# DelphinusLab/halo2-gpu-specific

Hardware: AMD Instinct MI355X
Metric: NTT Fr-ops/s @ k=24 (forward+inverse 2^24 BN254 Fr NTT; MSM G1-adds/s under 'msm') (higher is better)
Workload: dtype u32x8 (254-bit Montgomery, integer)

## Files before the change

### halo2-gpu-specific_amd/csrc/field.hpp

```cpp
#pragma once
#ifdef __HIPCC_RTC__
typedef unsigned char uint8_t;
typedef unsigned short uint16_t;
typedef unsigned int uint32_t;
typedef unsigned long uint64_t;
typedef int int32_t;
typedef long int64_t;
#else
#include <hip/hip_runtime.h>
#include <stdint.h>
#endif

namespace h2 {

struct FrParams {
    static constexpr uint32_t MOD[8] = {0xf0000001u, 0x43e1f593u, 0x79b97091u, 0x2833e848u,
                                        0x8181585du, 0xb85045b6u, 0xe131a029u, 0x30644e72u};
    static constexpr uint32_t MOD2[8] = {0xe0000002u, 0x87c3eb27u, 0xf372e122u, 0x5067d090u,
                                         0x0302b0bau, 0x70a08b6du, 0xc2634053u, 0x60c89ce5u};
    static constexpr uint32_t NMOD[8] = {0x0fffffffu, 0xbc1e0a6cu, 0x86468f6eu, 0xd7cc17b7u,
                                         0x7e7ea7a2u, 0x47afba49u, 0x1ece5fd6u, 0xcf9bb18du};
    static constexpr uint32_t PINV256[8] = {0xefffffffu, 0xc2e1f593u, 0x4c6911b3u, 0x6586864bu,
                                         0x99062391u, 0xe39a9828u, 0x0d8341b2u, 0x73f82f1du};
    static constexpr uint32_t INV = 0xefffffffu;
// ... 280 lines not shown
    u.l[0] = add_co(d.l[0], P::MOD2[0], cb);
#pragma unroll
    for (int i = 2; i < 8; i++) {
        d.l[i] = subb_co(a.l[i], b.l[i], ca);
        u.l[i - 1] = addc_co(d.l[i - 1], P::MOD2[i - 1], cb);
    }
    u.l[7] = addc_co(d.l[7], P::MOD2[7], cb);
#else
    uint64_t borrow = 0, c = 0;
#pragma unroll
    for (int i = 0; i < 8; i++) {
        uint64_t t = (uint64_t)a.l[i] - b.l[i] - borrow;
        d.l[i] = (uint32_t)t;
        borrow = (t >> 32) & 1;
    }
#pragma unroll
    for (int i = 0; i < 8; i++) {
        c += (uint64_t)d.l[i] + P::MOD2[i];
        u.l[i] = (uint32_t)c;
        c >>= 32;
    }
#endif
    return u;
}
template <class P>
H2_DEV Fp<P> fp_lazy_add_red(const Fp<P>& a, const Fp<P>& b) {
#ifdef H2_ASM_CHAINS
    Fp<P> s, t, r;
    uint64_t ca, cb;
    s.l[0] = add_co(a.l[0], b.l[0], ca);
    s.l[1] = addc_co(a.l[1], b.l[1], ca);
    t.l[0] = sub_co(s.l[0], P::MOD2[0], cb);
#pragma unroll
    for (int i = 2; i < 8; i++) {
        s.l[i] = addc_co(a.l[i], b.l[i], ca);
        t.l[i - 1] = subb_co(s.l[i - 1], P::MOD2[i - 1], cb);
    }
    t.l[7] = subb_co(s.l[7], P::MOD2[7], cb);
#pragma unroll
    for (int i = 0; i < 8; i++) r.l[i] = sel_co(t.l[i], s.l[i], cb);
    return r;
#else
    return fp_lazy_red2p(fp_lazy_add(a, b));
#endif
}
template <class P>
H2_DEV Fp<P> fp_lazy_sub_red(const Fp<P>& a, const Fp<P>& b) {
#ifdef H2_ASM_CHAINS
    Fp<P> d, u, r;
    uint64_t ca, cb;
    d.l[0] = sub_co(a.l[0], b.l[0], ca);
    d.l[1] = subb_co(a.l[1], b.l[1], ca);
    u.l[0] = add_co(d.l[0], P::MOD2[0], cb);
#pragma unroll
    for (int i = 2; i < 8; i++) {
        d.l[i] = subb_co(a.l[i], b.l[i], ca);
        u.l[i - 1] = addc_co(d.l[i - 1], P::MOD2[i - 1], cb);
    }
    u.l[7] = addc_co(d.l[7], P::MOD2[7], cb);
#pragma unroll
    for (int i = 0; i < 8; i++) r.l[i] = sel_co(d.l[i], u.l[i], ca);
    return r;
#else
    return fp_lazy_red2p(fp_lazy_sub(a, b));
#endif
}
template <class P>
H2_DEV Fp<P> fp_lazy_canon(const Fp<P>& a) {
    return fp_reduce_once(fp_lazy_red2p(a));
}

template <int CL>
struct alignas(16) FpChunk {
    uint32_t w[64 / CL];
};

H2_DEV void mad_acc(uint64_t& lo, uint32_t& hi, uint32_t a, uint32_t b) {
#if defined(H2_PORTABLE_MUL) || !defined(__HIP_DEVICE_COMPILE__)
    uint64_t p = (uint64_t)a * b;
    uint64_t s = lo + p;
    hi += (s < p) ? 1u : 0u;
    lo = s;
#else
    uint64_t carry;
    asm("v_mad_u64_u32 %0, %1, %2, %3, %0" : "+v"(lo), "=s"(carry) : "v"(a), "v"(b));
    asm("v_addc_co_u32 %0, %1, %0, 0, %1" : "+v"(hi), "+s"(carry));
#endif
}

template <class P>
__device__ __forceinline__ Fp<P> fp_mul_dev(const Fp<P>& a, const Fp<P>& b);
template <class P>
__device__ __forceinline__ Fp<P> fp_sqr_dev(const Fp<P>& a);
template <class P>
__device__ __forceinline__ Fp<P> fp_mul2_dev(const Fp<P>& a, const Fp<P>& b, const Fp<P>& c, const Fp<P>& d);
template <class P>
__device__ __forceinline__ Fp<P> fp_mul_wide_dev(const Fp<P>& a, const Fp<P>& b);
template <class P>
__device__ __forceinline__ Fp<P> fp_mul_const_dev(const Fp<P>& a, const Fp<P>& w, const Fp<P>& wq);
template <class P, int CL>
__device__ __forceinline__ Fp<P> fp_mul_chunk_dev(const Fp<P>& a, const FpChunk<CL>& t);
#if defined(__HIP_DEVICE_COMPILE__) && !defined(H2_PORTABLE_MUL)
#include "fp_mul_gen.hpp"
#endif

template <class P>
H2_DEV Fp<P> fp_mul(const Fp<P>& a, const Fp<P>& b) {
#if !defined(__HIP_DEVICE_COMPILE__)
    {
        typedef unsigned __int128 u128;
        uint64_t x[4], y[4], p[4];
        for (int i = 0; i < 4; i++) {
            x[i] = (uint64_t)a.l[2 * i] | ((uint64_t)a.l[2 * i + 1] << 32);
            y[i] = (uint64_t)b.l[2 * i] | ((uint64_t)b.l[2 * i + 1] << 32);
            p[i] = (uint64_t)P::MOD[2 * i] | ((uint64_t)P::MOD[2 * i + 1] << 32);
        }
        uint64_t inv = p[0];
        for (int i = 0; i < 6; i++) inv *= 2 - p[0] * inv;
        inv = 0 - inv;
        uint64_t t[6] = {0, 0, 0, 0, 0, 0};
        for (int i = 0; i < 4; i++) {
            u128 c = 0;
            for (int j = 0; j < 4; j++) {
                c += (u128)t[j] + (u128)x[j] * y[i];
                t[j] = (uint64_t)c;
                c >>= 64;
            }
            c += t[4];
            t[4] = (uint64_t)c;
            t[5] = (uint64_t)(c >> 64);
            const uint64_t m = t[0] * inv;
            c = ((u128)t[0] + (u128)m * p[0]) >> 64;
            for (int j = 1; j < 4; j++) {
                c += (u128)t[j] + (u128)m * p[j];
                t[j - 1] = (uint64_t)c;
                c >>= 64;
            }
            c += t[4];
            t[3] = (uint64_t)c;
            t[4] = t[5] + (uint64_t)(c >> 64);
        }
        Fp<P> r;
        for (int i = 0; i < 4; i++) {
            r.l[2 * i] = (uint32_t)t[i];
            r.l[2 * i + 1] = (uint32_t)(t[i] >> 32);
        }
        return fp_reduce_once(r);
    }
#elif !defined(H2_PORTABLE_MUL)
    return fp_mul_dev(a, b);
#endif
    Fp<P> r;
    uint64_t lo = 0;
    uint32_t hi = 0;
    uint32_t m[8];
#pragma unroll
    for (int i = 0; i < 8; i++) {
#pragma unroll
        for (int j = 0; j <= i; j++) mad_acc(lo, hi, a.l[j], b.l[i - j]);
#pragma unroll
        for (int j = 0; j < i; j++) mad_acc(lo, hi, m[j], P::MOD[i - j]);
        m[i] = (uint32_t)lo * P::INV;
        mad_acc(lo, hi, m[i], P::MOD[0]);
        lo = (lo >> 32) | ((uint64_t)hi << 32);
        hi = 0;
    }
#pragma unroll
    for (int i = 8; i < 16; i++) {
#pragma unroll
        for (int j = i - 7; j < 8; j++) mad_acc(lo, hi, a.l[j], b.l[i - j]);
#pragma unroll
        for (int j = i - 7; j < 8; j++) mad_acc(lo, hi, m[j], P::MOD[i - j]);
        r.l[i - 8] = (uint32_t)lo;
        lo = (lo >> 32) | ((uint64_t)hi << 32);
        hi = 0;
    }
    return fp_reduce_once(r);
}

template <class P>
H2_DEV Fp<P> fp_sqr(const Fp<P>& a) {
#if defined(__HIP_DEVICE_COMPILE__) && !defined(H2_PORTABLE_MUL) && !defined(H2_NO_SQR)
    return fp_sqr_dev(a);
#else
    return fp_mul(a, a);
#endif
}

template <class P>
H2_DEV Fp<P> fp_mul2(const Fp<P>& a, const Fp<P>& b, const Fp<P>& c, const Fp<P>& d) {
#if defined(__HIP_DEVICE_COMPILE__) && !defined(H2_PORTABLE_MUL) && !defined(H2_NO_MUL2)
    return fp_mul2_dev(a, b, c, d);
#else
    return fp_add(fp_mul(a, b), fp_mul(c, d));
#endif
}

template <class P>
H2_DEV Fp<P> fp_mul_wide(const Fp<P>& a, const Fp<P>& b) {
#if defined(__HIP_DEVICE_COMPILE__) && !defined(H2_PORTABLE_MUL)
    return fp_mul_wide_dev(a, b);
#else
    Fp<P> r;
    uint64_t lo = 0;
    uint32_t hi = 0;
    uint32_t m[8];
    for (int i = 0; i < 8; i++) {
        for (int j = 0; j <= i; j++) mad_acc(lo, hi, a.l[j], b.l[i - j]);
        for (int j = 0; j < i; j++) mad_acc(lo, hi, m[j], P::MOD[i - j]);
        m[i] = (uint32_t)lo * P::INV;
        mad_acc(lo, hi, m[i], P::MOD[0]);
        lo = (lo >> 32) | ((uint64_t)hi << 32);
        hi = 0;
    }
    for (int i = 8; i < 16; i++) {
        for (int j = i - 7; j < 8; j++) mad_acc(lo, hi, a.l[j], b.l[i - j]);
        for (int j = i - 7; j < 8; j++) mad_acc(lo, hi, m[j], P::MOD[i - j]);
        r.l[i - 8] = (uint32_t)lo;
        lo = (lo >> 32) | ((uint64_t)hi << 32);
        hi = 0;
    }
    return r;
#endif
}

template <class P>
H2_DEV Fp<P> fp_mul_const(const Fp<P>& x, const Fp<P>& w, const Fp<P>& wq) {
#if defined(__HIP_DEVICE_COMPILE__) && !defined(H2_PORTABLE_MUL)
    Fp<P> r = fp_mul_const_dev(x, w, wq);
    if (__builtin_expect(r.l[7] >= P::MOD2[7], 0)) r = fp_lazy_red2p(r);
    return r;
#else
    uint32_t q[8];
    {
        uint64_t lo = 0;
        uint32_t hi = 0;
        for (int i = 0; i < 15; i++) {
            for (int j = (i > 7 ? i - 7 : 0); j <= (i < 7 ? i : 7); j++) mad_acc(lo, hi, x.l[j], wq.l[i - j]);
            if (i >= 8) q[i - 8] = (uint32_t)lo;
            lo = (lo >> 32) | ((uint64_t)hi << 32);
            hi = 0;
        }
        q[7] = (uint32_t)lo;
    }
    Fp<P> r;
    uint64_t lo = 0;
    uint32_t hi = 0;
    for (int i = 0; i < 8; i++) {
        for (int j = 0; j <= i; j++) {
            mad_acc(lo, hi, x.l[j], w.l[i - j]);
            mad_acc(lo, hi, q[j], P::NMOD[i - j]);
        }
        r.l[i] = (uint32_t)lo;
        lo = (lo >> 32) | ((uint64_t)hi << 32);
        hi = 0;
    }
    return r;
#endif
}
template <class P>
H2_DEV void fp_const_pair(const Fp<P>& w_mont, Fp<P>& w_plain, Fp<P>& wq) {
    w_plain = fp_from_mont(w_mont);
    uint64_t lo = 0;
    uint32_t hi = 0;
    for (int i = 0; i < 8; i++) {
        for (int j = 0; j <= i; j++) mad_acc(lo, hi, w_mont.l[j], P::PINV256[i - j]);
        wq.l[i] = (uint32_t)lo;
        lo = (lo >> 32) | ((uint64_t)hi << 32);
        hi = 0;
    }
}

template <int CL, class P>
H2_DEV Fp<P> fp_mul_chunk(const Fp<P>& x, const FpChunk<CL>& t) {
#if defined(__HIP_DEVICE_COMPILE__) && !defined(H2_PORTABLE_MUL)
    return fp_mul_chunk_dev<P, CL>(x, t);
#else
    constexpr int NC = 8 / CL, NM = CL + 1;
    Fp<P> r;
    uint64_t lo = 0;
    uint32_t hi = 0;
    uint32_t m[NM];
    for (int i = 0; i < NM + 7; i++) {
        for (int j = 0; j < 8; j++) {
            const int l = i - j % CL;
            if (l >= 0 && l <= 7) mad_acc(lo, hi, x.l[j], t.w[l * NC + j / CL]);
        }
        for (int j = 0; j < NM && j < i; j++)
            if (i - j <= 7) mad_acc(lo, hi, m[j], P::MOD[i - j]);
        if (i < NM) {
            m[i] = (uint32_t)lo * P::INV;
            mad_acc(lo, hi, m[i], P::MOD[0]);
        } else {
            r.l[i - NM] = (uint32_t)lo;
        }
        lo = (lo >> 32) | ((uint64_t)hi << 32);
        hi = 0;
    }
    r.l[7] = (uint32_t)lo;
    return r;
#endif
}
template <int CL, class P>
H2_DEV void fp_chunk_table(const Fp<P>& w_mont, FpChunk<CL>& out) {
    constexpr int NC = 8 / CL;
    const Fp<P> w_plain = fp_from_mont(w_mont);
    for (int k = 0; k < NC; k++) {
        Fp<P> c;
        for (int l = 0; l < 8; l++) c.l[l] = P::CHUNK_POW[CL * k + CL - 1][l];
        const Fp<P> t = fp_mul(w_plain, c);
        for (int l = 0; l < 8; l++) out.w[l * NC + k] = t.l[l];
    }
}

template <class P>
H2_DEV Fp<P> fp_to_mont(const Fp<P>& canon) {
    Fp<P> rr;
#pragma unroll
    for (int i = 0; i < 8; i++) rr.l[i] = P::RR[i];
    return fp_reduce_once(fp_mul_wide(canon, rr));
}
template <class P>
H2_DEV Fp<P> fp_from_mont(const Fp<P>& a) {
    Fp<P> one = fp_zero<P>();
    one.l[0] = 1;
    return fp_reduce_once(fp_mul_wide(a, one));
}

template <class P>
H2_DEV Fp<P> fp_inv(const Fp<P>& a) {
    uint32_t u[8], v[8], r[8], s[8];
    uint32_t nz = 0;
#pragma unroll
    for (int i = 0; i < 8; i++) {
        u[i] = P::MOD[i];
        v[i] = a.l[i];
        r[i] = 0;
        s[i] = i == 0 ? 1u : 0u;
        nz |= a.l[i];
    }
    if (nz == 0) return a;
    uint32_t k = 0;
    auto halve = [](uint32_t* x) {
#pragma unroll
        for (int i = 0; i < 8; i++) x[i] = (x[i] >> 1) | (i < 7 ? x[i + 1] << 31 : 0u);
    };
    auto dbl = [](uint32_t* x) {
#pragma unroll
        for (int i = 7; i >= 0; i--) x[i] = (x[i] << 1) | (i ? x[i - 1] >> 31 : 0u);
    };
    auto sub = [](uint32_t* x, const uint32_t* y) {
        uint32_t bw = 0;
#pragma unroll
        for (int i = 0; i < 8; i++) {
            const uint32_t d = x[i] - y[i], b1 = x[i] < y[i] ? 1u : 0u, e = d - bw, b2 = d < bw ? 1u : 0u;
            x[i] = e;
            bw = b1 | b2;
        }
    };
    auto add = [](uint32_t* x, const uint32_t* y) {
        uint32_t cy = 0;
#pragma unroll
        for (int i = 0; i < 8; i++) {
            const uint32_t t = x[i] + y[i], c1 = t < y[i] ? 1u : 0u, e = t + cy, c2 = e < cy ? 1u : 0u;
            x[i] = e;
            cy = c1 | c2;
        }
    };
    auto greater = [](const uint32_t* x, const uint32_t* y) {
#pragma unroll
        for (int i = 7; i >= 0; i--)
            if (x[i] != y[i]) return x[i] > y[i];
        return false;
    };
    for (;;) {
        uint32_t vnz = 0;
#pragma unroll
        for (int i = 0; i < 8; i++) vnz |= v[i];
        if (vnz == 0) break;
        if ((u[0] & 1) == 0) {
            halve(u);
            dbl(s);
        } else if ((v[0] & 1) == 0) {
            halve(v);
            dbl(r);
        } else if (greater(u, v)) {
            sub(u, v);
            halve(u);
            add(r, s);
            dbl(s);
        } else {
            sub(v, u);
            halve(v);
            add(s, r);
            dbl(r);
        }
        k++;
    }
    Fp<P> x;
    {
        uint32_t d[8];
        uint64_t bw = 0;
#pragma unroll
        for (int i = 0; i < 8; i++) {
            uint64_t e = (uint64_t)r[i] - P::MOD[i] - bw;
            d[i] = (uint32_t)e;
            bw = (e >> 32) & 1;
        }
        uint64_t bw2 = 0;
#pragma unroll
        for (int i = 0; i < 8; i++) {
            const uint32_t rr = bw ? r[i] : d[i];
            uint64_t e = (uint64_t)P::MOD[i] - rr - bw2;
            x.l[i] = (uint32_t)e;
            bw2 = (e >> 32) & 1;
        }
    }
    x = fp_reduce_once(x);
    for (uint32_t i = k; i < 512; i++) x = fp_dbl(x);
    return x;
}

template <class P>
H2_DEV Fp<P> fp_pow_u32(const Fp<P>& a, uint32_t e) {
    if (e == 0) return fp_one<P>();
    Fp<P> acc = a;
    for (int i = 30 - __builtin_clz(e); i >= 0; i--) {
        acc = fp_sqr(acc);
        if ((e >> i) & 1) acc = fp_mul(acc, a);
    }
    return acc;
}

}
```

### halo2-gpu-specific_amd/csrc/ntt_pass.hip

```cpp
#include <stdexcept>

#include "ntt_pass.hpp"

namespace h2 {

__device__ __forceinline__ void tw_store(Fr* out, uint32_t i, const Fr& w_mont, uint32_t pair) {
    if (!pair) {
        fp_store(out + i, w_mont);
        return;
    }
    if (pair == 2) {
        TwChunk t;
        fp_chunk_table(w_mont, t);
        uint4* const q = reinterpret_cast<uint4*>(out) + (size_t)i * TW_CHUNK_Q;
#pragma unroll
        for (uint32_t k = 0; k < TW_CHUNK_Q; k++) q[k] = make_uint4(t.w[4 * k], t.w[4 * k + 1], t.w[4 * k + 2], t.w[4 * k + 3]);
        return;
    }
    Fr w, q;
    fp_const_pair(w_mont, w, q);
    fp_store(out + 2 * (size_t)i, w);
    fp_store(out + 2 * (size_t)i + 1, q);
}

// ... 70 lines not shown
    hi[i] = make_uint4(v.l[4], v.l[5], v.l[6], v.l[7]);
}

__device__ __forceinline__ Fr store_twiddle(const PassArgs& a, const Fr& y, const uint32_t entry) {
    const uint4* const q = reinterpret_cast<const uint4*>(a.nx_tab) + (size_t)entry * TW_CHUNK_Q;
    TwChunk t;
#pragma unroll
    for (uint32_t k = 0; k < TW_CHUNK_Q; k++) {
        const uint4 v = q[k];
        t.w[4 * k] = v.x; t.w[4 * k + 1] = v.y; t.w[4 * k + 2] = v.z; t.w[4 * k + 3] = v.w;
    }
    return fp_mul_chunk(y, t);
}

template <bool RADIX4, bool NLAST = false, bool ST = false>
__global__ void __launch_bounds__(512, 4) k_ntt_pass(PassArgs a) {
    constexpr bool CW = RADIX4;
    static_assert(!ST || NLAST || !RADIX4, "a last pass stores the transform's output");
    const bool is_last = NLAST ? false : a.is_last != 0;
    auto tmul = [](const Fr& x, const Fr& w) -> Fr { return fp_mul_wide(x, w); };
    const uint32_t B = a.B, R = 1u << B, log_c = a.log_c, C = 1u << log_c;
    const uint32_t zskip = a.zskip;
    uint4* t_lo = h2_smem;
    uint4* t_hi = t_lo + (R << log_c);
    uint4* w_lo = t_hi + (R << log_c);
    uint4* w_hi = w_lo + (R >> 1) + (CW ? 0 : 1);
    uint4* q_lo = w_hi + (R >> 1);
    uint4* q_hi = q_lo + (R >> 1);
    struct Tw {
        Fr w, q;
    };
    auto tw_get = [&](uint32_t i) __attribute__((always_inline)) -> Tw {
        Tw t;
        t.w = lds_get(w_lo, w_hi, i);
        if constexpr (CW) t.q = lds_get(q_lo, q_hi, i);
        return t;
    };
    auto bmul = [](const Fr& x, const Tw& t) __attribute__((always_inline)) -> Fr {
        if constexpr (CW) return fp_mul_const(x, t.w, t.q);
        else return fp_mul_wide(x, t.w);
    };
    const uint32_t nthreads = blockDim.x;
    const uint32_t tid = threadIdx.x;
    const Fr* const in_p = a.batch ? a.in_b[blockIdx.y] : a.in;
    Fr* const out_p = a.batch ? a.out_b[blockIdx.y] : a.out;
    const uint32_t n_mask = (a.log_n >= 32) ? 0xffffffffu : ((1u << a.log_n) - 1);

    for (uint32_t i = tid; i < (R >> 1); i += nthreads) {
        if constexpr (CW) {
            lds_put(w_lo, w_hi, i, fp_load(a.tw_bfly + 2 * i));
            lds_put(q_lo, q_hi, i, fp_load(a.tw_bfly + 2 * i + 1));
        } else {
            lds_put(w_lo, w_hi, i, fp_load(a.tw_bfly + i));
        }
    }

    const uint32_t tile_id = blockIdx.x;
    const uint32_t total = R << log_c;

    uint32_t base = 0, K_uniform = 0;
    const uint32_t S = 1u << a.s_log;
    if (!is_last) {
        uint32_t chunks_per_hi = S >> log_c;
        uint32_t hi = tile_id / chunks_per_hi, lo0 = (tile_id % chunks_per_hi) << log_c;
        base = (hi << (B + a.s_log)) + lo0;
        K_uniform = hi_to_K(hi, a);
    }

    constexpr uint32_t NE = RADIX4 ? 4 : 2;
    for (uint32_t e0 = tid; e0 < total; e0 += NE * nthreads) {
        uint32_t rho[NE], col[NE], idx[NE], Kk[NE];
        bool live[NE];
        Fr x[NE];
#pragma unroll
        for (uint32_t q = 0; q < NE; q++) {
            const uint32_t e = e0 + q * nthreads;
            if (!is_last) {
                col[q] = e & (C - 1);
                rho[q] = (e >> log_c) & (R - 1);
                idx[q] = base + (rho[q] << a.s_log) + col[q];
                Kk[q] = K_uniform;
            } else {
                rho[q] = e & (R - 1);
                col[q] = (e >> B) & (C - 1);
                Kk[q] = (tile_id << log_c) + col[q];
                idx[q] = (K_to_hi(Kk[q], a) << B) + rho[q];
            }
            live[q] = e < total && !(zskip && rho[q] >= (R >> zskip));
        }
#pragma unroll
        for (uint32_t q = 0; q < NE; q++) {
            x[q] = fp_zero<FrParams>();
            if (live[q] && idx[q] < a.in_len) x[q] = fp_load(in_p + idx[q]);
        }
        if (a.has_pre3) {
#pragma unroll
            for (uint32_t q = 0; q < NE; q++) {
                const uint32_t m = idx[q] % 3;
                Fr w;
#pragma unroll
                for (int l = 0; l < 8; l++) w.l[l] = m == 1 ? a.pre3[1].l[l] : a.pre3[2].l[l];
                if (m != 0) x[q] = tmul(x[q], w);
            }
        }
        const bool pre_scale = a.scale_mode == 1u && a.nprev == 0;
        if ((a.nprev != 0 && !a.tw_applied) || pre_scale) {
            if (!NLAST && a.tw_direct != nullptr && !pre_scale) {
#pragma unroll
                for (uint32_t q0 = 0; q0 < NE; q0 += 2) {
                    Fr w[2];
#pragma unroll
                    for (uint32_t q = 0; q < 2; q++) w[q] = fp_load(a.tw_direct + ((Kk[q0 + q] << B) | rho[q0 + q]));
#pragma unroll
                    for (uint32_t q = 0; q < 2; q++) x[q0 + q] = tmul(x[q0 + q], w[q]);
                }
            } else if (a.log_n <= LO_BITS && !pre_scale) {
#pragma unroll
                for (uint32_t q = 0; q < NE; q++) {
                    const uint32_t ex = (uint32_t)(((uint64_t)rho[q] * Kk[q]) << a.s_log) & n_mask;
                    x[q] = tmul(x[q], fp_load(a.tw_lo + ex));
                }
            } else {
                const Fr* const two_lo = pre_scale ? a.sc_lo : a.tw_lo;
                const Fr* const two_hi = pre_scale ? a.sc_hi : a.tw_hi;
#pragma unroll
                for (uint32_t q0 = 0; q0 < NE; q0 += 2) {
                    Fr wl[2], wh[2];
#pragma unroll
                    for (uint32_t q = 0; q < 2; q++) {
                        const uint32_t ex = pre_scale ? (idx[q0 + q] & n_mask)
                                                      : ((uint32_t)(((uint64_t)rho[q0 + q] * Kk[q0 + q]) << a.s_log) & n_mask);
                        wl[q] = fp_load(two_lo + (ex & ((1u << LO_BITS) - 1)));
                        wh[q] = fp_load(two_hi + (ex >> LO_BITS));
                    }
#pragma unroll
                    for (uint32_t q = 0; q < 2; q++) x[q0 + q] = tmul(x[q0 + q], fp_mul(wl[q], wh[q]));
                }
            }
        }
#pragma unroll
        for (uint32_t q = 0; q < NE; q++) {
            const uint32_t e = e0 + q * nthreads;
            const uint32_t r_q = is_last ? (e & (R - 1)) : ((e >> log_c) & (R - 1));
            const uint32_t c_q = is_last ? ((e >> B) & (C - 1)) : (e & (C - 1));
            if (e >= total || (zskip && r_q >= (R >> zskip))) continue;
            if (zskip) {
                for (uint32_t m = 0; m < (1u << zskip); m++) lds_put(t_lo, t_hi, ((bitrev(r_q, B) | m) << log_c) + c_q, x[q]);
            } else {
                lds_put(t_lo, t_hi, (bitrev(r_q, B) << log_c) + c_q, x[q]);
            }
        }
    }
    __syncthreads();

    uint32_t s0 = zskip;
    if constexpr (RADIX4) {
        const uint32_t nunits = total >> 2;
        auto round4 = [&](const uint32_t s) __attribute__((always_inline)) {
            const uint32_t h = 1u << s;
            const uint32_t log_per = (B - 2 + log_c) - s;
            const bool by_r = s != 0 && log_per >= 6 && (nthreads & 63) == 0;
            for (uint32_t t = tid; t < nunits; t += nthreads) {
                uint32_t c, r, p;
                if (by_r) {
                    r = t >> log_per;
                    const uint32_t j = t & ((1u << log_per) - 1);
                    c = j & (C - 1);
                    p = ((j >> log_c) << (s + 2)) | r;
                } else {
                    c = t & (C - 1);
                    const uint32_t b = t >> log_c;
                    r = b & (h - 1);
                    p = ((b >> s) << (s + 2)) | r;
                }
                const uint32_t i0 = (p << log_c) + c, step = h << log_c;
                Fr x0 = lds_get(t_lo, t_hi, i0), x1 = lds_get(t_lo, t_hi, i0 + step);
                Fr x2 = lds_get(t_lo, t_hi, i0 + 2 * step), x3 = lds_get(t_lo, t_hi, i0 + 3 * step);
                const bool unit = s == 0 || (by_r && r == 0);
                x0 = fp_lazy_red2p(x0);
                x2 = fp_lazy_red2p(x2);
                if (!unit) {
                    const Tw wa = tw_get(r << (B - 1 - s));
                    x1 = bmul(x1, wa);
                    x3 = bmul(x3, wa);
                } else {
                    x1 = fp_lazy_red2p(x1);
                    x3 = fp_lazy_red2p(x3);
                }
                const Fr y0 = fp_lazy_add_red(x0, x1), y1 = fp_lazy_sub_red(x0, x1);
                Fr y2 = fp_lazy_add(x2, x3), y3 = fp_lazy_sub(x2, x3);
                y2 = unit ? fp_lazy_red2p(y2) : bmul(y2, tw_get(r << (B - 2 - s)));
                y3 = bmul(y3, tw_get((r + h) << (B - 2 - s)));
                lds_put(t_lo, t_hi, i0, fp_lazy_add(y0, y2));
                lds_put(t_lo, t_hi, i0 + 2 * step, fp_lazy_sub(y0, y2));
                lds_put(t_lo, t_hi, i0 + step, fp_lazy_add(y1, y3));
                lds_put(t_lo, t_hi, i0 + 3 * step, fp_lazy_sub(y1, y3));
            }
            __syncthreads();
        };
        for (; s0 + 1 < B; s0 += 2) round4(s0);
    }
    const uint32_t nbf = total >> 1;
    for (uint32_t s = s0; s < B; s++) {
        const uint32_t h = 1u << s;
        const uint32_t log_per = (B - 1 + log_c) - s;
        const bool by_r = s != 0 && log_per >= 6 && (nthreads & 63) == 0;
        for (uint32_t t = tid; t < nbf; t += nthreads) {
            uint32_t c, r, i;
            if (by_r) {
                r = t >> log_per;
                uint32_t j = t & ((1u << log_per) - 1);
                c = j & (C - 1);
                i = ((j >> log_c) << (s + 1)) | r;
            } else {
                c = t & (C - 1);
                uint32_t b = t >> log_c;
                r = b & (h - 1);
                i = ((b >> s) << (s + 1)) | r;
            }
            const uint32_t iu = (i << log_c) + c, iv = ((i + h) << log_c) + c;
            Fr u = lds_get(t_lo, t_hi, iu), v = lds_get(t_lo, t_hi, iv);
            const bool skip = s == 0 || (by_r && r == 0);
            u = fp_lazy_red2p(u);
            v = skip ? fp_lazy_red2p(v) : bmul(v, tw_get(r << (B - 1 - s)));
            lds_put(t_lo, t_hi, iu, fp_lazy_add(u, v));
            lds_put(t_lo, t_hi, iv, fp_lazy_sub(u, v));
        }
        __syncthreads();
    }

    for (uint32_t e0 = tid; e0 < total; e0 += NE * nthreads) {
        Fr y[NE];
        uint32_t idx[NE];
#pragma unroll
        for (uint32_t q = 0; q < NE; q++) {
            const uint32_t e = e0 + q * nthreads;
            const uint32_t c = e & (C - 1), k = (e >> log_c) & (R - 1);
            if (!is_last)
                idx[q] = base + (k << a.s_log) + c;
            else
                idx[q] = ((tile_id << log_c) + c) + (k << a.t_log);
            y[q] = lds_get(t_lo, t_hi, (k << log_c) + c);
        }
        if (is_last && a.scale_mode == 2u) {
#pragma unroll
            for (uint32_t q = 0; q < NE; q++) {
                const uint32_t i = idx[q] & n_mask;
                const Fr w = fp_mul(fp_load(a.sc_lo + (i & ((1u << LO_BITS) - 1))), fp_load(a.sc_hi + (i >> LO_BITS)));
                y[q] = fp_reduce_once(fp_mul_wide(y[q], w));
            }
        } else if (is_last && a.has_post3 && !a.hi_scaled) {
#pragma unroll
            for (uint32_t q = 0; q < NE; q++) {
                const uint32_t m = idx[q] % 3;
                Fr w;
#pragma unroll
                for (int l = 0; l < 8; l++) w.l[l] = m == 0 ? a.post3[0].l[l] : (m == 1 ? a.post3[1].l[l] : a.post3[2].l[l]);
                y[q] = fp_reduce_once(fp_mul_wide(y[q], w));
            }
        } else if (is_last) {
#pragma unroll
            for (uint32_t q = 0; q < NE; q++) y[q] = fp_lazy_canon(y[q]);
        }
        if constexpr (ST) {
#pragma unroll
            for (uint32_t q = 0; q < NE; q++) {
                const uint32_t e = e0 + q * nthreads;
                const uint32_t rho_n = (idx[q] >> a.nx_s_log) & ((1u << a.nx_B) - 1);
                const uint32_t K_n = K_uniform | (((e >> log_c) & (R - 1)) << a.t_log);
                if (e < total) y[q] = store_twiddle(a, y[q], (rho_n << a.nx_t_log) | K_n);
            }
        }
#pragma unroll
        for (uint32_t q = 0; q < NE; q++)
            if (e0 + q * nthreads < total) fp_store(out_p + idx[q], y[q]);
    }
}

static constexpr uint32_t PASS8_TW_LDS = 32;
static constexpr uint32_t PASS8_LDS = ((256u << 2) * 2 + PASS8_TW_LDS * TW_CHUNK_Q) * sizeof(uint4);
static_assert(4 * PASS8_LDS <= 160u * 1024, "four workgroups of k_ntt_pass8 per CU");
template <bool NLAST, bool ST = false>
__global__ void __launch_bounds__(256, 4) k_ntt_pass8(PassArgs a) {
    static_assert(!ST || NLAST, "a last pass stores the transform's output");
    constexpr uint32_t B = 8, R = 1u << B, log_c = 2, C = 1u << log_c;
    auto tmul = [](const Fr& x, const Fr& w) -> Fr { return fp_mul_wide(x, w); };
    uint4* t_lo = h2_smem;
    uint4* t_hi = t_lo + (R << log_c);
    uint4* w_pl = t_hi + (R << log_c);
    const uint4* const tw_tab = reinterpret_cast<const uint4*>(a.tw_chunk);
    using Tw = TwChunk;
    auto tw_unpack = [](Tw& t, const uint32_t k, const uint4 v) __attribute__((always_inline)) {
        t.w[4 * k] = v.x; t.w[4 * k + 1] = v.y; t.w[4 * k + 2] = v.z; t.w[4 * k + 3] = v.w;
    };
    static_assert((R >> 1) / PASS8_TW_LDS == 4, "the stage pairs before the last read the indices that are multiples of 4");
    auto tw_get = [&](const uint32_t i, const bool mem) __attribute__((always_inline)) -> Tw {
        Tw t;
#pragma unroll
        for (uint32_t k = 0; k < TW_CHUNK_Q; k++)
            tw_unpack(t, k, mem ? tw_tab[(size_t)i * TW_CHUNK_Q + k] : w_pl[k * PASS8_TW_LDS + (i >> 2)]);
        return t;
    };
    auto bmul = [](const Fr& x, const Tw& t) __attribute__((always_inline)) -> Fr { return fp_mul_chunk(x, t); };
    auto unit4 = [&](Fr& x0, Fr& x1, Fr& x2, Fr& x3, const uint32_t s, const uint32_t r, const bool unit, const Tw* w3 = nullptr) __attribute__((always_inline)) {
        const uint32_t h = 1u << s;
        const bool mem = s == B - 2;
        x0 = fp_lazy_red2p(x0);
        x2 = fp_lazy_red2p(x2);
        if (!unit) {
            const Tw wa = tw_get(r << (B - 1 - s), mem);
            x1 = bmul(x1, wa);
            x3 = bmul(x3, wa);
        } else {
            x1 = fp_lazy_red2p(x1);
            x3 = fp_lazy_red2p(x3);
        }
        const Fr y0 = fp_lazy_add_red(x0, x1), y1 = fp_lazy_sub_red(x0, x1);
        Fr y2 = fp_lazy_add(x2, x3), y3 = fp_lazy_sub(x2, x3);
        y2 = unit ? fp_lazy_red2p(y2) : bmul(y2, tw_get(r << (B - 2 - s), mem));
        y3 = bmul(y3, w3 ? *w3 : tw_get((r + h) << (B - 2 - s), mem));
        x0 = fp_lazy_add(y0, y2);
        x1 = fp_lazy_add(y1, y3);
        x2 = fp_lazy_sub(y0, y2);
        x3 = fp_lazy_sub(y1, y3);
    };
    auto unit_of = [](const uint32_t tid, const uint32_t s, uint32_t& i0, uint32_t& r, bool& unit) __attribute__((always_inline)) {
        const uint32_t h = 1u << s, log_per = (B - 2 + log_c) - s;
        const bool by_r = s != 0 && log_per >= 6;
        uint32_t c, p;
        if (by_r) {
            r = tid >> log_per;
            const uint32_t j = tid & ((1u << log_per) - 1);
            c = j & (C - 1);
            p = ((j >> log_c) << (s + 2)) | r;
        } else {
            c = tid & (C - 1);
            const uint32_t b = tid >> log_c;
            r = b & (h - 1);
            p = ((b >> s) << (s + 2)) | r;
        }
        i0 = (p << log_c) + c;
        unit = s == 0 || (by_r && r == 0);
    };
    const uint32_t tid = threadIdx.x;
    auto round4 = [&](const uint32_t s) __attribute__((always_inline)) {
        uint32_t i0, r;
        bool unit;
        unit_of(tid, s, i0, r, unit);
        const uint32_t step = (1u << s) << log_c;
        Fr x0 = lds_get(t_lo, t_hi, i0), x1 = lds_get(t_lo, t_hi, i0 + step);
        Fr x2 = lds_get(t_lo, t_hi, i0 + 2 * step), x3 = lds_get(t_lo, t_hi, i0 + 3 * step);
        unit4(x0, x1, x2, x3, s, r, unit);
        lds_put(t_lo, t_hi, i0, x0);
        lds_put(t_lo, t_hi, i0 + 2 * step, x2);
        lds_put(t_lo, t_hi, i0 + step, x1);
        lds_put(t_lo, t_hi, i0 + 3 * step, x3);
        __syncthreads();
    };
    const bool is_last = NLAST ? false : a.is_last != 0;
    const uint32_t n_mask = (a.log_n >= 32) ? 0xffffffffu : ((1u << a.log_n) - 1);

#pragma unroll
    for (uint32_t g = tid; g < PASS8_TW_LDS * TW_CHUNK_Q; g += 256)
        w_pl[(g % TW_CHUNK_Q) * PASS8_TW_LDS + g / TW_CHUNK_Q] = tw_tab[(size_t)(g / TW_CHUNK_Q) * 4 * TW_CHUNK_Q + g % TW_CHUNK_Q];

    Tw tw64;
#pragma unroll
    for (uint32_t k = 0; k < TW_CHUNK_Q; k++) tw_unpack(tw64, k, tw_tab[(R >> 2) * TW_CHUNK_Q + k]);

    constexpr uint32_t NE = 4;
    {
        const uint32_t tile_id = blockIdx.x;
        const Fr* const in_p = a.batch ? a.in_b[blockIdx.y] : a.in;
        Fr* const out_p = a.batch ? a.out_b[blockIdx.y] : a.out;
        uint32_t base = 0, K_uniform = 0;
        if (!is_last) {
            const uint32_t chunks_per_hi = (1u << a.s_log) >> log_c;
            const uint32_t hi = tile_id / chunks_per_hi, lo0 = (tile_id % chunks_per_hi) << log_c;
            base = (hi << (B + a.s_log)) + lo0;
            K_uniform = hi_to_K(hi, a);
        }

        {
            uint32_t rho[NE], col[NE], idx[NE], Kk[NE];
            Fr x[NE];
#pragma unroll
            for (uint32_t q = 0; q < NE; q++) {
                if (!is_last) {
                    col[q] = tid & (C - 1);
                    rho[q] = bitrev(tid >> log_c, B - 2) + (q << (B - 2));
                    idx[q] = base + (rho[q] << a.s_log) + col[q];
                    Kk[q] = K_uniform;
                } else {
                    rho[q] = (tid & 63) + (q << (B - 2));
                    col[q] = tid >> 6;
                    Kk[q] = (tile_id << log_c) + col[q];
                    idx[q] = (K_to_hi(Kk[q], a) << B) + rho[q];
                }
            }
#pragma unroll
            for (uint32_t q = 0; q < NE; q++) {
                x[q] = fp_zero<FrParams>();
                if (idx[q] < a.in_len) x[q] = fp_load(in_p + idx[q]);
            }
            if (a.has_pre3) {
#pragma unroll
                for (uint32_t q = 0; q < NE; q++) {
                    const uint32_t m = idx[q] % 3;
                    Fr w;
#pragma unroll
                    for (int l = 0; l < 8; l++) w.l[l] = m == 1 ? a.pre3[1].l[l] : a.pre3[2].l[l];
                    if (m != 0) x[q] = tmul(x[q], w);
                }
            }
            const bool pre_scale = a.scale_mode == 1u && a.nprev == 0;
            if ((a.nprev != 0 && !a.tw_applied) || pre_scale) {
                if (!NLAST && a.tw_direct != nullptr && !pre_scale) {
#pragma unroll
                    for (uint32_t q0 = 0; q0 < NE; q0 += 2) {
                        Fr w[2];
#pragma unroll
                        for (uint32_t q = 0; q < 2; q++) w[q] = fp_load(a.tw_direct + ((Kk[q0 + q] << B) | rho[q0 + q]));
#pragma unroll
                        for (uint32_t q = 0; q < 2; q++) x[q0 + q] = tmul(x[q0 + q], w[q]);
                    }
                } else if (a.log_n <= LO_BITS && !pre_scale) {
#pragma unroll
                    for (uint32_t q = 0; q < NE; q++) {
                        const uint32_t ex = (uint32_t)(((uint64_t)rho[q] * Kk[q]) << a.s_log) & n_mask;
                        x[q] = tmul(x[q], fp_load(a.tw_lo + ex));
                    }
                } else {
                    const Fr* const two_lo = pre_scale ? a.sc_lo : a.tw_lo;
                    const Fr* const two_hi = pre_scale ? a.sc_hi : a.tw_hi;
#pragma unroll
                    for (uint32_t q0 = 0; q0 < NE; q0 += 2) {
                        Fr wl[2], wh[2];
#pragma unroll
                        for (uint32_t q = 0; q < 2; q++) {
                            const uint32_t ex = pre_scale ? (idx[q0 + q] & n_mask)
                                                          : ((uint32_t)(((uint64_t)rho[q0 + q] * Kk[q0 + q]) << a.s_log) & n_mask);
                            wl[q] = fp_load(two_lo + (ex & ((1u << LO_BITS) - 1)));
                            wh[q] = fp_load(two_hi + (ex >> LO_BITS));
                        }
#pragma unroll
                        for (uint32_t q = 0; q < 2; q++) x[q0 + q] = tmul(x[q0 + q], fp_mul(wl[q], wh[q]));
                    }
                }
            }
            const uint32_t b = is_last ? bitrev(tid & 63, B - 2) : (tid >> log_c);
            const uint32_t i0 = (b << (2 + log_c)) + (is_last ? (tid >> 6) : (tid & (C - 1)));
            unit4(x[0], x[2], x[1], x[3], 0, 0, true, &tw64);
            lds_put(t_lo, t_hi, i0, x[0]);
            lds_put(t_lo, t_hi, i0 + 2 * C, x[1]);
            lds_put(t_lo, t_hi, i0 + C, x[2]);
            lds_put(t_lo, t_hi, i0 + 3 * C, x[3]);
        }
        __syncthreads();
        round4(2);
        round4(4);

        Fr y[NE];
        {
            uint32_t i0, r;
            bool unit;
            unit_of(tid, 6, i0, r, unit);
#pragma unroll
            for (uint32_t q = 0; q < NE; q++) y[q] = lds_get(t_lo, t_hi, i0 + q * (R << log_c) / NE);
            unit4(y[0], y[1], y[2], y[3], 6, r, unit);
        }
        uint32_t idx[NE];
#pragma unroll
        for (uint32_t q = 0; q < NE; q++) {
            const uint32_t c = tid & (C - 1), k = (tid >> log_c) + q * (R / NE);
            if (!is_last)
                idx[q] = base + (k << a.s_log) + c;
            else
                idx[q] = ((tile_id << log_c) + c) + (k << a.t_log);
        }
        if (is_last && a.scale_mode == 2u) {
#pragma unroll
            for (uint32_t q = 0; q < NE; q++) {
                const uint32_t i = idx[q] & n_mask;
                const Fr w = fp_mul(fp_load(a.sc_lo + (i & ((1u << LO_BITS) - 1))), fp_load(a.sc_hi + (i >> LO_BITS)));
                y[q] = fp_reduce_once(fp_mul_wide(y[q], w));
            }
        } else if (is_last && a.has_post3 && !a.hi_scaled) {
#pragma unroll
            for (uint32_t q = 0; q < NE; q++) {
                const uint32_t m = idx[q] % 3;
                Fr w;
#pragma unroll
                for (int l = 0; l < 8; l++) w.l[l] = m == 0 ? a.post3[0].l[l] : (m == 1 ? a.post3[1].l[l] : a.post3[2].l[l]);
                y[q] = fp_reduce_once(fp_mul_wide(y[q], w));
            }
        } else if (is_last) {
#pragma unroll
            for (uint32_t q = 0; q < NE; q++) y[q] = fp_lazy_canon(y[q]);
        }
        if constexpr (ST) {
            const uint32_t rho_n = (base >> a.nx_s_log) & ((1u << a.nx_B) - 1);
#pragma unroll
            for (uint32_t q = 0; q < NE; q++) {
                const uint32_t K_n = K_uniform | (((tid >> log_c) + q * (R / NE)) << a.t_log);
                y[q] = store_twiddle(a, y[q], (rho_n << a.nx_t_log) | K_n);
            }
        }
#pragma unroll
        for (uint32_t q = 0; q < NE; q++) fp_store(out_p + idx[q], y[q]);
    }
}

using PassFn = void (*)(PassArgs);
static const PassFn pass_fn[H2_NTT_KERNEL_COUNT] = {
    k_ntt_pass8<true>,
    k_ntt_pass8<false>,
    k_ntt_pass<true, true>,
    k_ntt_pass<true, false>,
    k_ntt_pass<false>,
};
static const PassFn pass_fn_st[H2_NTT_KERNEL_COUNT] = {
    k_ntt_pass8<true, true>, nullptr, k_ntt_pass<true, true, true>, nullptr, k_ntt_pass<false, false, true>,
};

void ntt_pass_launch(int device, NttKernel kernel, const PassArgs& a, uint32_t cnt, uint32_t threads, hipStream_t stream) {
    const uint32_t R = 1u << a.B, C = 1u << a.log_c;
    const uint32_t ntiles = (1u << a.log_n) / (R * C);
    const size_t lds = kernel != NK_R2 ? ((size_t)R * C + R) * sizeof(Fr) : ((size_t)R * C + (R >> 1) + 2) * sizeof(Fr);
    if (lds > 64 * 1024) {
        static bool raised[64] = {};
        if (device < 0 || device >= 64 || !raised[device]) {
            for (const PassFn f : {pass_fn[NK_R4_DP], pass_fn[NK_R4], pass_fn[NK_R2], pass_fn_st[NK_R4_DP], pass_fn_st[NK_R2]})
                H2_HIP(hipFuncSetAttribute((const void*)f, hipFuncAttributeMaxDynamicSharedMemorySize, 160 * 1024));
            if (device >= 0 && device < 64) raised[device] = true;
        }
    }
    const bool pass8 = kernel == NK_PASS8_DP || kernel == NK_PASS8;
    const PassFn fn = a.nx_tab ? pass_fn_st[kernel] : pass_fn[kernel];
    if (!fn) throw std::runtime_error("ntt_pass_launch: a last pass has no next pass to multiply for");
    hipLaunchKernelGGL(fn, dim3(ntiles, cnt), dim3(threads), pass8 ? (size_t)PASS8_LDS : lds, stream, a);
}

static dim3 fill_grid(uint32_t count) { return dim3((count + 255) / 256); }

void ntt_fill_pow(Fr* out, const Fr& base, uint32_t mul, uint32_t count, uint32_t form, hipStream_t stream) {
    if (count) hipLaunchKernelGGL(k_pow_table, fill_grid(count), dim3(256), 0, stream, out, base, mul, count, form);
}

void ntt_fill_direct(Fr* out, const Fr& base, uint32_t kbits, uint32_t s_log, uint32_t log_n, uint32_t count, uint32_t form,
                     hipStream_t stream) {
    hipLaunchKernelGGL(k_direct_table, fill_grid(count), dim3(256), 0, stream, out, base, kbits, s_log, log_n, count, form);
}

void ntt_fill_last(Fr* out, const Fr& base, uint32_t bits, uint32_t log_n, const Fr* d, hipStream_t stream) {
    hipLaunchKernelGGL(k_last_table, fill_grid(1u << log_n), dim3(256), 0, stream, out, base, bits, log_n, d ? *d : base,
                       d ? 1u : 0u, 0u);
}

void ntt_fill_scaled(Fr* out, const Fr* in, const Fr& d, uint32_t count, hipStream_t stream) {
    hipLaunchKernelGGL(k_scale_table, fill_grid(count), dim3(256), 0, stream, out, in, d, count);
}

}
```

Measured before the change: 425.7 billion.

## Prefetch twiddles ahead of compute and split radix-4 unit into mul/add phases

Splits the radix-4 butterfly helper into a multiply phase and an add phase so the next-pass store twiddle table can be loaded in between. Store-side twiddle multiplies now software-pipeline the next element's chunk-table loads around the current multiply, fenced with sched_barrier. The LDS twiddle copy is changed from a loop to one preloaded word per lane, written after the input loads. The first direct-twiddle pair is loaded early, and a specialised first butterfly skips redundant lazy reductions when inputs are already reduced. This aims to hide global-memory latency, at the cost of more register pressure and constrained scheduling.

After: 433.4 billion, median of 6. 1.8% higher.

```diff
diff --git a/halo2-gpu-specific_amd/csrc/field.hpp b/halo2-gpu-specific_amd/csrc/field.hpp
--- a/halo2-gpu-specific_amd/csrc/field.hpp
+++ b/halo2-gpu-specific_amd/csrc/field.hpp
@@ -606,6 +606,22 @@
 #endif
 }
 template <int CL, class P>
+H2_DEV void fp_lazy_first_pair(Fp<P>& x0, Fp<P>& x1, Fp<P>& x2, Fp<P>& x3, const FpChunk<CL>& w3, const bool red) {
+    if (red) {
+        x0 = fp_lazy_red2p(x0);
+        x1 = fp_lazy_red2p(x1);
+        x2 = fp_lazy_red2p(x2);
+        x3 = fp_lazy_red2p(x3);
+    }
+    const Fp<P> y0 = fp_lazy_add_red(x0, x1), y1 = fp_lazy_sub_red(x0, x1);
+    const Fp<P> y2 = fp_lazy_red2p(fp_lazy_add(x2, x3));
+    const Fp<P> y3 = fp_mul_chunk(fp_lazy_sub(x2, x3), w3);
+    x0 = fp_lazy_add(y0, y2);
+    x1 = fp_lazy_add(y1, y3);
+    x2 = fp_lazy_sub(y0, y2);
+    x3 = fp_lazy_sub(y1, y3);
+}
+template <int CL, class P>
 H2_DEV void fp_chunk_table(const Fp<P>& w_mont, FpChunk<CL>& out) {
     constexpr int NC = 8 / CL;
     const Fp<P> w_plain = fp_from_mont(w_mont);
diff --git a/halo2-gpu-specific_amd/csrc/ntt_pass.hip b/halo2-gpu-specific_amd/csrc/ntt_pass.hip
--- a/halo2-gpu-specific_amd/csrc/ntt_pass.hip
+++ b/halo2-gpu-specific_amd/csrc/ntt_pass.hip
@@ -396,7 +396,7 @@
         return t;
     };
     auto bmul = [](const Fr& x, const Tw& t) __attribute__((always_inline)) -> Fr { return fp_mul_chunk(x, t); };
-    auto unit4 = [&](Fr& x0, Fr& x1, Fr& x2, Fr& x3, const uint32_t s, const uint32_t r, const bool unit, const Tw* w3 = nullptr) __attribute__((always_inline)) {
+    auto unit4_mul = [&](Fr& x0, Fr& x1, Fr& x2, Fr& x3, const uint32_t s, const uint32_t r, const bool unit) __attribute__((always_inline)) {
         const uint32_t h = 1u << s;
         const bool mem = s == B - 2;
         x0 = fp_lazy_red2p(x0);
@@ -412,7 +412,14 @@
         const Fr y0 = fp_lazy_add_red(x0, x1), y1 = fp_lazy_sub_red(x0, x1);
         Fr y2 = fp_lazy_add(x2, x3), y3 = fp_lazy_sub(x2, x3);
         y2 = unit ? fp_lazy_red2p(y2) : bmul(y2, tw_get(r << (B - 2 - s), mem));
-        y3 = bmul(y3, w3 ? *w3 : tw_get((r + h) << (B - 2 - s), mem));
+        y3 = bmul(y3, tw_get((r + h) << (B - 2 - s), mem));
+        x0 = y0;
+        x1 = y1;
+        x2 = y2;
+        x3 = y3;
+    };
+    auto unit4_add = [](Fr& x0, Fr& x1, Fr& x2, Fr& x3) __attribute__((always_inline)) {
+        const Fr y0 = x0, y1 = x1, y2 = x2, y3 = x3;
         x0 = fp_lazy_add(y0, y2);
         x1 = fp_lazy_add(y1, y3);
         x2 = fp_lazy_sub(y0, y2);
@@ -444,7 +451,8 @@
         const uint32_t step = (1u << s) << log_c;
         Fr x0 = lds_get(t_lo, t_hi, i0), x1 = lds_get(t_lo, t_hi, i0 + step);
         Fr x2 = lds_get(t_lo, t_hi, i0 + 2 * step), x3 = lds_get(t_lo, t_hi, i0 + 3 * step);
-        unit4(x0, x1, x2, x3, s, r, unit);
+        unit4_mul(x0, x1, x2, x3, s, r, unit);
+        unit4_add(x0, x1, x2, x3);
         lds_put(t_lo, t_hi, i0, x0);
         lds_put(t_lo, t_hi, i0 + 2 * step, x2);
         lds_put(t_lo, t_hi, i0 + step, x1);
@@ -454,9 +462,8 @@
     const bool is_last = NLAST ? false : a.is_last != 0;
     const uint32_t n_mask = (a.log_n >= 32) ? 0xffffffffu : ((1u << a.log_n) - 1);
 
-#pragma unroll
-    for (uint32_t g = tid; g < PASS8_TW_LDS * TW_CHUNK_Q; g += 256)
-        w_pl[(g % TW_CHUNK_Q) * PASS8_TW_LDS + g / TW_CHUNK_Q] = tw_tab[(size_t)(g / TW_CHUNK_Q) * 4 * TW_CHUNK_Q + g % TW_CHUNK_Q];
+    static_assert(PASS8_TW_LDS * TW_CHUNK_Q == 256, "one word of the LDS copy per lane");
+    const uint4 w_fill = tw_tab[(size_t)(tid / TW_CHUNK_Q) * 4 * TW_CHUNK_Q + tid % TW_CHUNK_Q];
 
     Tw tw64;
 #pragma unroll
@@ -497,6 +504,15 @@
                 x[q] = fp_zero<FrParams>();
                 if (idx[q] < a.in_len) x[q] = fp_load(in_p + idx[q]);
             }
+            const bool pre_scale = a.scale_mode == 1u && a.nprev == 0;
+            const bool direct = !NLAST && a.nprev != 0 && !a.tw_applied && a.tw_direct != nullptr && !pre_scale;
+            Fr wd[2];
+            if (direct) {
+#pragma unroll
+                for (uint32_t q = 0; q < 2; q++) wd[q] = fp_load(a.tw_direct + ((Kk[q] << B) | rho[q]));
+            }
+            __builtin_amdgcn_sched_barrier(0);
+            w_pl[(tid % TW_CHUNK_Q) * PASS8_TW_LDS + tid / TW_CHUNK_Q] = w_fill;
             if (a.has_pre3) {
 #pragma unroll
                 for (uint32_t q = 0; q < NE; q++) {
@@ -507,17 +523,15 @@
                     if (m != 0) x[q] = tmul(x[q], w);
                 }
             }
-            const bool pre_scale = a.scale_mode == 1u && a.nprev == 0;
             if ((a.nprev != 0 && !a.tw_applied) || pre_scale) {
-                if (!NLAST && a.tw_direct != nullptr && !pre_scale) {
-#pragma unroll
-                    for (uint32_t q0 = 0; q0 < NE; q0 += 2) {
-                        Fr w[2];
-#pragma unroll
-                        for (uint32_t q = 0; q < 2; q++) w[q] = fp_load(a.tw_direct + ((Kk[q0 + q] << B) | rho[q0 + q]));
-#pragma unroll
-                        for (uint32_t q = 0; q < 2; q++) x[q0 + q] = tmul(x[q0 + q], w[q]);
-                    }
+                if (direct) {
+                    Fr w[2];
+#pragma unroll
+                    for (uint32_t q = 0; q < 2; q++) w[q] = fp_load(a.tw_direct + ((Kk[2 + q] << B) | rho[2 + q]));
+#pragma unroll
+                    for (uint32_t q = 0; q < 2; q++) x[q] = tmul(x[q], wd[q]);
+#pragma unroll
+                    for (uint32_t q = 0; q < 2; q++) x[2 + q] = tmul(x[2 + q], w[q]);
                 } else if (a.log_n <= LO_BITS && !pre_scale) {
 #pragma unroll
                     for (uint32_t q = 0; q < NE; q++) {
@@ -544,7 +558,7 @@
             }
             const uint32_t b = is_last ? bitrev(tid & 63, B - 2) : (tid >> log_c);
             const uint32_t i0 = (b << (2 + log_c)) + (is_last ? (tid >> 6) : (tid & (C - 1)));
-            unit4(x[0], x[2], x[1], x[3], 0, 0, true, &tw64);
+            fp_lazy_first_pair(x[0], x[2], x[1], x[3], tw64, !(a.nprev != 0 || pre_scale));
             lds_put(t_lo, t_hi, i0, x[0]);
             lds_put(t_lo, t_hi, i0 + 2 * C, x[1]);
             lds_put(t_lo, t_hi, i0 + C, x[2]);
@@ -555,13 +569,28 @@
         round4(4);
 
         Fr y[NE];
+        const uint4* nx_q = nullptr;
+        size_t nx_step = 0;
+        if constexpr (ST) {
+            const uint32_t rho_n = (base >> a.nx_s_log) & ((1u << a.nx_B) - 1);
+            const uint32_t K_n = K_uniform | ((tid >> log_c) << a.t_log);
+            nx_q = reinterpret_cast<const uint4*>(a.nx_tab) + (size_t)((rho_n << a.nx_t_log) | K_n) * TW_CHUNK_Q;
+            nx_step = (size_t)((R / NE) << a.t_log) * TW_CHUNK_Q;
+        }
+        Tw nx_t;
         {
             uint32_t i0, r;
             bool unit;
             unit_of(tid, 6, i0, r, unit);
 #pragma unroll
             for (uint32_t q = 0; q < NE; q++) y[q] = lds_get(t_lo, t_hi, i0 + q * (R << log_c) / NE);
-            unit4(y[0], y[1], y[2], y[3], 6, r, unit);
+            unit4_mul(y[0], y[1], y[2], y[3], 6, r, unit);
+            if constexpr (ST) {
+#pragma unroll
+                for (uint32_t k = 0; k < TW_CHUNK_Q; k++) tw_unpack(nx_t, k, nx_q[k]);
+                __builtin_amdgcn_sched_barrier(0);
+            }
+            unit4_add(y[0], y[1], y[2], y[3]);
         }
         uint32_t idx[NE];
 #pragma unroll
@@ -593,11 +622,23 @@
             for (uint32_t q = 0; q < NE; q++) y[q] = fp_lazy_canon(y[q]);
         }
         if constexpr (ST) {
-            const uint32_t rho_n = (base >> a.nx_s_log) & ((1u << a.nx_B) - 1);
-#pragma unroll
-            for (uint32_t q = 0; q < NE; q++) {
-                const uint32_t K_n = K_uniform | (((tid >> log_c) + q * (R / NE)) << a.t_log);
-                y[q] = store_twiddle(a, y[q], (rho_n << a.nx_t_log) | K_n);
+            constexpr uint32_t PF = TW_CHUNK_Q / 2;
+#pragma unroll
+            for (uint32_t q = 0; q < NE; q++) {
+                uint4 pf[PF];
+                if (q + 1 < NE) {
+#pragma unroll
+                    for (uint32_t k = 0; k < PF; k++) pf[k] = nx_q[(q + 1) * nx_step + k];
+                    __builtin_amdgcn_sched_barrier(0);
+                }
+                y[q] = fp_mul_chunk(y[q], nx_t);
+                if (q + 1 < NE) {
+                    __builtin_amdgcn_sched_barrier(0);
+#pragma unroll
+                    for (uint32_t k = PF; k < TW_CHUNK_Q; k++) tw_unpack(nx_t, k, nx_q[(q + 1) * nx_step + k]);
+#pragma unroll
+                    for (uint32_t k = 0; k < PF; k++) tw_unpack(nx_t, k, pf[k]);
+                }
             }
         }
 #pragma unroll
```
